# Lapis-Hong/wide_deep

Measured on NVIDIA H100. Metric: CTR examples/sec (train step), higher is better.
Workload: dtype bf16x3 (fp32 operands split into bf16 hi+lo, 3 tensor-core products, fp32 accumulate; 2^-16)

## Files before the change

### wide_deep_b200/csrc/gemm_bf16.cu

```cuda
#include <cuda.h>
#include <stdlib.h>

#include <algorithm>
#include <type_traits>

#include "common.cuh"
#include "gemm.cuh"
#include "wgmma_ptx.cuh"

namespace wd {

namespace {

constexpr int QBM = 128;
constexpr int QBN = 128;
constexpr int QNST = 3;
constexpr int QBK = 64;
constexpr int Q_THREADS = 384;

struct QMaps {
    CUtensorMap a_hi[kMaxSegs], a_lo[kMaxSegs];
    CUtensorMap b_hi, b_lo;
};
struct QSegs { int n; int k[kMaxSegs]; int koff[kMaxSegs]; };

__device__ unsigned long long g_probe[32 * 8];
__device__ __forceinline__ unsigned long long gtime() { unsigned long long t; asm volatile("mov.u64 %0, %globaltimer;" : "=l"(t)); return t; }
#define PROBE(i) do { if (probe >= 0 && blockIdx.x == 0 && (threadIdx.x & 127) == 0) g_probe[probe * 8 + (i)] = gtime(); } while (0)

template <int MODE>
__global__ void __launch_bounds__(Q_THREADS, 1) tc_gemm_bf16_kernel(const __grid_constant__ QMaps maps, const QSegs segs, int M, int N, int ktot,
                                                                   int ksplit_len, int nsplit, Epi ep, int probe) {
    extern __shared__ uint8_t smem_raw[];
    uint8_t* base = reinterpret_cast<uint8_t*>((reinterpret_cast<uintptr_t>(smem_raw) + 1023) & ~uintptr_t(1023));
    constexpr bool A_MN = MODE == EPI_WGRAD;
    constexpr bool B_MN = MODE == EPI_FWD || MODE == EPI_WGRAD;
    constexpr int A_BYTES = QBM * 128, B_BYTES = QBN * 128;
    constexpr int STAGE_BYTES = 2 * (A_BYTES + B_BYTES);
    auto a_hi = [&](int s) { return base + s * STAGE_BYTES; };
    auto a_lo = [&](int s) { return base + s * STAGE_BYTES + A_BYTES; };
    auto b_hi = [&](int s) { return base + s * STAGE_BYTES + 2 * A_BYTES; };
    auto b_lo = [&](int s) { return base + s * STAGE_BYTES + 2 * A_BYTES + B_BYTES; };
    uint64_t* bars = reinterpret_cast<uint64_t*>(base + QNST * STAGE_BYTES);
    uint64_t* full = bars; uint64_t* empty = bars + QNST;
    float* epi_vec = reinterpret_cast<float*>(base + QNST * STAGE_BYTES + 64);

    const int warp = threadIdx.x >> 5, lane = threadIdx.x & 31, wg = threadIdx.x >> 7;
    const int tiles_n = (N + QBN - 1) / QBN, tiles_m = (M + QBM - 1) / QBM;
    const int ntiles = tiles_n * tiles_m * nsplit;
    int nkb_all = 0;
    for (int s = 0; s < segs.n; ++s) nkb_all += (segs.k[s] + QBK - 1) / QBK;
    auto tile_range = [&](int tile, int& m0, int& n0, int& z, int& kbeg, int& nkb) {
        z = tile / (tiles_n * tiles_m);
        int r = tile % (tiles_n * tiles_m);
        m0 = (r / tiles_n) * QBM;
        n0 = (r % tiles_n) * QBN;
        kbeg = 0;
        nkb = nkb_all;
        if (MODE == EPI_WGRAD) {
            kbeg = z * ksplit_len;
            int kend = min(ktot, kbeg + ksplit_len);
            nkb = kend > kbeg ? (kend - kbeg + QBK - 1) / QBK : 0;
        }
    };

    if (threadIdx.x == 0) {
        for (int s = 0; s < QNST; ++s) { mbar_init(&full[s], 1); mbar_init(&empty[s], 8); }
        asm volatile("fence.mbarrier_init.release.cluster;" ::: "memory");
    }
    __syncthreads();

    if (wg == 0) {
        reg_dealloc<40>();
        PROBE(0);
        if (warp == 0 && lane == 0) {
            int g = 0;
            for (int tile = blockIdx.x; tile < ntiles; tile += gridDim.x) {
                int m0, n0, z, kbeg, nkb;
                tile_range(tile, m0, n0, z, kbeg, nkb);
                int seg = 0, kin = 0;
                for (int kb = 0; kb < nkb; ++kb, ++g) {
                    const int s = g % QNST, it = g / QNST;
                    if (it > 0) mbar_wait(&empty[s], (it - 1) & 1);
                    int ka, kbcoord;
                    if (MODE == EPI_WGRAD) { ka = kbeg + kb * QBK; kbcoord = ka; }
                    else {
                        if (kin >= segs.k[seg]) { ++seg; kin = 0; }
                        ka = kin; kbcoord = segs.koff[seg] + kin;
                        kin += QBK;
                    }
                    mbar_expect_tx(&full[s], 2 * (A_BYTES + B_BYTES));
                    if (!A_MN) {
                        tma_load_2d(a_hi(s), &maps.a_hi[seg], &full[s], ka, m0);
                        tma_load_2d(a_lo(s), &maps.a_lo[seg], &full[s], ka, m0);
                    } else {
#pragma unroll
                        for (int i = 0; i < QBM / 64; ++i) {
                            tma_load_2d(a_hi(s) + i * 8192, &maps.a_hi[seg], &full[s], m0 + 64 * i, ka);
                            tma_load_2d(a_lo(s) + i * 8192, &maps.a_lo[seg], &full[s], m0 + 64 * i, ka);
                        }
                    }
                    if (!B_MN) {
                        tma_load_2d(b_hi(s), &maps.b_hi, &full[s], kbcoord, n0);
                        tma_load_2d(b_lo(s), &maps.b_lo, &full[s], kbcoord, n0);
                    } else {
#pragma unroll
                        for (int i = 0; i < QBN / 64; ++i) {
                            tma_load_2d(b_hi(s) + i * 8192, &maps.b_hi, &full[s], n0 + 64 * i, kbcoord);
                            tma_load_2d(b_lo(s) + i * 8192, &maps.b_lo, &full[s], n0 + 64 * i, kbcoord);
                        }
                    }
                }
            }
        }
    } else {
        reg_alloc<232>();
        const int cw = wg - 1, cwarp = warp - 4;
        constexpr uint32_t a_step = A_MN ? 2048u : 32u, b_step = B_MN ? 2048u : 32u;
        constexpr int TA = A_MN ? 1 : 0, TB = B_MN ? 1 : 0;
        float d[QBN / 2];
        int g = 0, use = 0;
        for (int tile = blockIdx.x; tile < ntiles; tile += gridDim.x) {
            int m0, n0, z, kbeg, nkb;
            tile_range(tile, m0, n0, z, kbeg, nkb);
            if (nkb == 0) {
#pragma unroll
                for (int i = 0; i < QBN / 2; ++i) d[i] = 0.f;
            }
            const int ct = threadIdx.x - 128;
            float pre[2] = {0.f, 0.f};
            if (MODE == EPI_FWD) {
#pragma unroll
                for (int i = 0; i < 2; ++i) {
                    const int v = ct + 256 * i, c = n0 + (v & 127);
                    const bool in = c < ep.n_logical;
                    if (v < 128) pre[i] = in ? __ldg(ep.bias + c) : 0.f;
                    else if (v < 256) pre[i] = (in && ep.bn) ? __ldg(ep.gamma + c) * 0.99950037468777f : 1.f;
                    else if (v < 384) pre[i] = (in && ep.bn) ? __ldg(ep.beta + c) : 0.f;
                }
            }
            int prev = -1;
            for (int kb = 0; kb < nkb; ++kb, ++g) {
                const int s = g % QNST, it = g / QNST;
                mbar_wait(&full[s], it & 1);
                if (g == 0) PROBE(1);
                const uint32_t sa_hi = smem_u32(a_hi(s)) + cw * 8192, sa_lo = smem_u32(a_lo(s)) + cw * 8192;
                const uint32_t sb_hi = smem_u32(b_hi(s)), sb_lo = smem_u32(b_lo(s));
                wgmma_fence();
#pragma unroll
                for (int k = 0; k < QBK / 16; ++k) {
                    const uint64_t da_hi = A_MN ? make_desc_mn(sa_hi + k * a_step) : make_desc(sa_hi + k * a_step);
                    const uint64_t da_lo = A_MN ? make_desc_mn(sa_lo + k * a_step) : make_desc(sa_lo + k * a_step);
                    const uint64_t db_hi = B_MN ? make_desc_mn(sb_hi + k * b_step) : make_desc(sb_hi + k * b_step);
                    const uint64_t db_lo = B_MN ? make_desc_mn(sb_lo + k * b_step) : make_desc(sb_lo + k * b_step);
                    wgmma_bf16<TA, TB>(d, da_lo, db_hi, (kb > 0 || k > 0) ? 1u : 0u);
                    wgmma_bf16<TA, TB>(d, da_hi, db_lo, 1u);
                    wgmma_bf16<TA, TB>(d, da_hi, db_hi, 1u);
                }
                wgmma_commit();
                if (prev >= 0) {
                    wgmma_wait<1>();
                    if (lane == 0) mbar_arrive(&empty[prev]);
                }
                prev = s;
            }
            wgmma_wait<0>();
            if (prev >= 0 && lane == 0) mbar_arrive(&empty[prev]);
            if (cwarp == 0) PROBE(use == 0 ? 2 : 3);
            const float* ev = epi_vec + (use & 1) * 384;
            if (MODE == EPI_FWD) {
                epi_vec[(use & 1) * 384 + ct] = pre[0];
                if (ct < 128) epi_vec[(use & 1) * 384 + ct + 256] = pre[1];
                bar_sync(1, 256);
            }

            const int r0 = m0 + cw * 64 + (warp & 3) * 16 + (lane >> 2);
            const int cq = 2 * (lane & 3);
            auto epilogue = [&](auto relu) {
                constexpr bool RELU = decltype(relu)::value;
                uint32_t qh[2][2] = {}, ql[2][2] = {};
#pragma unroll
                for (int j = 0; j < QBN / 8; ++j) {
                    const int c = n0 + 8 * j + cq;
                    if (n0 + 8 * j < N) {
                        if (MODE == EPI_FWD) {
                            const bool in0 = c < ep.n_logical, in1 = c + 1 < ep.n_logical;
                            const int cl = 8 * j + cq;
                            const float b0 = ev[cl], b1 = ev[cl + 1], g0 = ev[128 + cl], g1 = ev[129 + cl], e0 = ev[256 + cl], e1 = ev[257 + cl];
#pragma unroll
                            for (int hh = 0; hh < 2; ++hh) {
                                const int r = r0 + 8 * hh;
                                if (r >= M) continue;
                                const bool rv = r < ep.m_valid;
                                float a0 = 0.f, a1 = 0.f, h0 = 0.f, h1 = 0.f;
                                if (rv && in0) { a0 = RELU ? fmaxf(d[4 * j + 2 * hh] + b0, 0.f) : act_fwd(ep.act, d[4 * j + 2 * hh] + b0); h0 = fmaf(a0, g0, e0); }
                                if (rv && in1) { a1 = RELU ? fmaxf(d[4 * j + 2 * hh + 1] + b1, 0.f) : act_fwd(ep.act, d[4 * j + 2 * hh + 1] + b1); h1 = fmaf(a1, g1, e1); }
                                const int64_t o = (int64_t)r * ep.ldh + c;
                                if (ep.A_out != ep.H_out) *reinterpret_cast<float2*>(ep.A_out + o) = make_float2(a0, a1);
                                if (ep.H_out) *reinterpret_cast<float2*>(ep.H_out + o) = make_float2(h0, h1);
                                split_pair(h0, h1, qh[j & 1][hh], ql[j & 1][hh]);
                            }
                            if (j & 1) {
                                const int q = lane & 3, src = (lane & ~3) + 2 * (q & 1);
                                const int64_t cp = n0 + 16 * (j >> 1) + 4 * q;
#pragma unroll
                                for (int hh = 0; hh < 2; ++hh) {
                                    uint2 vh, vl;
                                    const uint32_t h0a = __shfl_sync(0xffffffffu, qh[0][hh], src), h1a = __shfl_sync(0xffffffffu, qh[1][hh], src);
                                    const uint32_t h0b = __shfl_sync(0xffffffffu, qh[0][hh], src + 1), h1b = __shfl_sync(0xffffffffu, qh[1][hh], src + 1);
                                    const uint32_t l0a = __shfl_sync(0xffffffffu, ql[0][hh], src), l1a = __shfl_sync(0xffffffffu, ql[1][hh], src);
                                    const uint32_t l0b = __shfl_sync(0xffffffffu, ql[0][hh], src + 1), l1b = __shfl_sync(0xffffffffu, ql[1][hh], src + 1);
                                    vh.x = q < 2 ? h0a : h1a; vh.y = q < 2 ? h0b : h1b;
                                    vl.x = q < 2 ? l0a : l1a; vl.y = q < 2 ? l0b : l1b;
                                    const int r = r0 + 8 * hh;
                                    if (r >= M) continue;
                                    const int64_t o = (int64_t)r * ep.ldh + cp;
                                    *reinterpret_cast<uint2*>(ep.Hs_hi + o) = vh;
                                    *reinterpret_cast<uint2*>(ep.Hs_lo + o) = vl;
                                }
                            }
                        } else {
                            float* Cb = ep.C + (MODE == EPI_WGRAD ? (int64_t)z * ep.split_stride : 0);
#pragma unroll
                            for (int hh = 0; hh < 2; ++hh) {
                                const int r = r0 + 8 * hh;
                                if (r >= M) continue;
                                float2* pc = reinterpret_cast<float2*>(Cb + (int64_t)r * ep.ldc + c);
                                float2 o = make_float2(d[4 * j + 2 * hh], d[4 * j + 2 * hh + 1]);
                                if (MODE == EPI_STORE && ep.accumulate) { const float2 p = *pc; o.x += p.x; o.y += p.y; }
                                *pc = o;
                            }
                        }
                    }
                }
            };
            if (MODE == EPI_FWD && ep.act == WD_ACT_RELU) epilogue(std::true_type{});
            else epilogue(std::false_type{});
            if (cwarp == 0) PROBE(use == 0 ? 4 : 5);
            ++use;
        }
    }
}

int g_probe_slot = 0;

template <int MODE>
int launch_q(WdModel* m, const QMaps& maps, const QSegs& segs, int M, int N, int ktot, int splits, int ksplit_len, const Epi& ep) {
    constexpr int smem = QNST * 2 * (QBM * 128 + QBN * 128) + 1024 + 64 + 2 * 384 * 4;
    static bool configured = false;
    static int num_sms = 0;
    if (!configured) {
        WD_CUDA(cudaFuncSetAttribute(tc_gemm_bf16_kernel<MODE>, cudaFuncAttributeMaxDynamicSharedMemorySize, smem));
        WD_CUDA(cudaDeviceGetAttribute(&num_sms, cudaDevAttrMultiProcessorCount, m->device));
        configured = true;
    }
    const int nsplit = MODE == EPI_WGRAD ? splits : 1;
    const int ntiles = ((N + QBN - 1) / QBN) * ((M + QBM - 1) / QBM) * nsplit;
    static const bool probe_on = getenv("WD_GEMM_PROBE") != nullptr;
    const int probe = probe_on ? (g_probe_slot++ & 31) : -1;
    tc_gemm_bf16_kernel<MODE><<<ntiles < num_sms ? ntiles : num_sms, Q_THREADS, smem, m->stream>>>(maps, segs, M, N, ktot, ksplit_len, nsplit, ep, probe);
    m->launches++;
    WD_CUDA(cudaGetLastError());
    return WD_OK;
}

}

extern "C" int wd_debug_gemm_probe(unsigned long long* out) {
    cudaDeviceSynchronize();
    cudaError_t e = cudaMemcpyFromSymbol(out, g_probe, sizeof(unsigned long long) * 32 * 8);
    g_probe_slot = 0;
    return e == cudaSuccess ? 0 : -1;
}

int tc_gemm_bf16(WdModel* m, int mode, const GemmA& A, const GemmB& B, int M, int N, const Epi& ep, int splits, int ksplit_len) {
    constexpr CUtensorMapDataType BF16 = CU_TENSOR_MAP_DATA_TYPE_BFLOAT16;
    if (N % 32 != 0 || A.n > kMaxSegs || !B.hi || !B.lo) { set_error("bf16 GEMM engine: unsupported operands"); return WD_EUNSUPPORTED; }
    QMaps maps;
    QSegs segs{};
    segs.n = A.n;
    int rc, ktot = 0;
    const bool a_mn = mode == EPI_WGRAD, b_mn = mode == EPI_FWD || mode == EPI_WGRAD;
    for (int s = 0; s < A.n; ++s) {
        if (!A.hi[s] || !A.lo[s]) { set_error("bf16 GEMM engine: operand without hi/lo copies"); return WD_EINVAL; }
        if (!a_mn) {
            if ((rc = make_tensor_map(&maps.a_hi[s], BF16, A.hi[s], M, A.k[s], A.ld[s], QBM))) return rc;
            if ((rc = make_tensor_map(&maps.a_lo[s], BF16, A.lo[s], M, A.k[s], A.ld[s], QBM))) return rc;
        } else {
            if ((rc = make_tensor_map(&maps.a_hi[s], BF16, A.hi[s], A.k[s], M, A.ld[s], 64))) return rc;
            if ((rc = make_tensor_map(&maps.a_lo[s], BF16, A.lo[s], A.k[s], M, A.ld[s], 64))) return rc;
        }
        segs.k[s] = A.k[s]; segs.koff[s] = ktot;
        ktot += A.k[s];
    }
    for (int s = A.n; s < kMaxSegs; ++s) { maps.a_hi[s] = maps.a_hi[0]; maps.a_lo[s] = maps.a_lo[0]; }
    if (!b_mn) {
        if ((rc = make_tensor_map(&maps.b_hi, BF16, B.hi, N, ktot, B.ld, QBN))) return rc;
        if ((rc = make_tensor_map(&maps.b_lo, BF16, B.lo, N, ktot, B.ld, QBN))) return rc;
    } else {
        if ((rc = make_tensor_map(&maps.b_hi, BF16, B.hi, ktot, N, B.ld, 64))) return rc;
        if ((rc = make_tensor_map(&maps.b_lo, BF16, B.lo, ktot, N, B.ld, 64))) return rc;
    }
    if (mode == EPI_WGRAD) ksplit_len = (ksplit_len + QBK - 1) / QBK * QBK;
    if (mode == EPI_FWD && (!ep.Hs_hi || !ep.Hs_lo)) { set_error("bf16 GEMM engine: epilogue without hi/lo outputs"); return WD_EINVAL; }
    if (mode == EPI_FWD) return launch_q<EPI_FWD>(m, maps, segs, M, N, ktot, splits, ksplit_len, ep);
    if (mode == EPI_STORE) return launch_q<EPI_STORE>(m, maps, segs, M, N, ktot, splits, ksplit_len, ep);
    return launch_q<EPI_WGRAD>(m, maps, segs, M, N, ktot, splits, ksplit_len, ep);
}

}
```

### wide_deep_b200/csrc/wgmma_ptx.cuh

```cuda
#pragma once
#include <cuda.h>
#include <stdint.h>

namespace wd {

__device__ __forceinline__ uint32_t smem_u32(const void* p) { return (uint32_t)__cvta_generic_to_shared(p); }
__device__ __forceinline__ void mbar_init(uint64_t* bar, uint32_t count) {
    asm volatile("mbarrier.init.shared::cta.b64 [%0], %1;" ::"r"(smem_u32(bar)), "r"(count));
}
__device__ __forceinline__ void mbar_expect_tx(uint64_t* bar, uint32_t bytes) {
    asm volatile("mbarrier.arrive.expect_tx.shared::cta.b64 _, [%0], %1;" ::"r"(smem_u32(bar)), "r"(bytes) : "memory");
}
__device__ __forceinline__ void mbar_arrive(uint64_t* bar) {
    asm volatile("mbarrier.arrive.shared::cta.b64 _, [%0];" ::"r"(smem_u32(bar)) : "memory");
}
__device__ __forceinline__ void mbar_wait(uint64_t* bar, uint32_t parity) {
    asm volatile(
        "{\n\t.reg .pred p;\n\t"
        "WAIT_LOOP:\n\t"
        "mbarrier.try_wait.parity.shared::cta.b64 p, [%0], %1;\n\t"
        "@p bra WAIT_DONE;\n\t"
        "bra WAIT_LOOP;\n\t"
        "WAIT_DONE:\n\t}" ::"r"(smem_u32(bar)), "r"(parity) : "memory");
}
__device__ __forceinline__ void tma_load_2d(void* dst, const CUtensorMap* map, uint64_t* bar, int c0, int c1) {
    asm volatile("cp.async.bulk.tensor.2d.shared::cluster.global.mbarrier::complete_tx::bytes [%0], [%1, {%3, %4}], [%2];"
                 ::"r"(smem_u32(dst)), "l"(reinterpret_cast<uint64_t>(map)), "r"(smem_u32(bar)), "r"(c0), "r"(c1) : "memory");
}

__device__ __forceinline__ void bar_sync(int id, int n) { asm volatile("bar.sync %0, %1;" ::"r"(id), "r"(n) : "memory"); }

template <int N> __device__ __forceinline__ void reg_dealloc() { asm volatile("setmaxnreg.dec.sync.aligned.u32 %0;" ::"n"(N)); }
template <int N> __device__ __forceinline__ void reg_alloc() { asm volatile("setmaxnreg.inc.sync.aligned.u32 %0;" ::"n"(N)); }

__device__ __forceinline__ void wgmma_fence() { asm volatile("wgmma.fence.sync.aligned;" ::: "memory"); }
__device__ __forceinline__ void wgmma_commit() { asm volatile("wgmma.commit_group.sync.aligned;" ::: "memory"); }
template <int N> __device__ __forceinline__ void wgmma_wait() { asm volatile("wgmma.wait_group.sync.aligned %0;" ::"n"(N) : "memory"); }

__device__ __forceinline__ uint64_t make_desc(uint32_t saddr) {
    uint64_t d = 0;
    d |= (uint64_t)((saddr >> 4) & 0x3FFF);
    d |= (uint64_t)1 << 16;
    d |= (uint64_t)(1024 >> 4) << 32;
    d |= (uint64_t)1 << 62;
    return d;
}

__device__ __forceinline__ uint64_t make_desc_mn(uint32_t saddr) {
    uint64_t d = 0;
    d |= (uint64_t)((saddr >> 4) & 0x3FFF);
    d |= (uint64_t)(8192 >> 4) << 16;
    d |= (uint64_t)(1024 >> 4) << 32;
    d |= (uint64_t)1 << 62;
    return d;
}

template <int TA, int TB>
__device__ __forceinline__ void wgmma_bf16(float (&d)[64], uint64_t desc_a, uint64_t desc_b, uint32_t accumulate) {
    asm volatile(
        "{\n\t.reg .pred p;\n\tsetp.ne.b32 p, %66, 0;\n\t"
        "wgmma.mma_async.sync.aligned.m64n128k16.f32.bf16.bf16 {"
        "%0, %1, %2, %3, %4, %5, %6, %7, %8, %9, %10, %11, %12, %13, %14, %15, %16, %17, %18, %19, %20, %21, %22, %23, %24, %25, "
        "%26, %27, %28, %29, %30, %31, %32, %33, %34, %35, %36, %37, %38, %39, %40, %41, %42, %43, %44, %45, %46, %47, %48, %49, "
        "%50, %51, %52, %53, %54, %55, %56, %57, %58, %59, %60, %61, %62, %63}, "
        "%64, %65, p, 1, 1, %67, %68;\n\t}"
        : "+f"(d[0]), "+f"(d[1]), "+f"(d[2]), "+f"(d[3]), "+f"(d[4]), "+f"(d[5]), "+f"(d[6]), "+f"(d[7]),
          "+f"(d[8]), "+f"(d[9]), "+f"(d[10]), "+f"(d[11]), "+f"(d[12]), "+f"(d[13]), "+f"(d[14]), "+f"(d[15]),
          "+f"(d[16]), "+f"(d[17]), "+f"(d[18]), "+f"(d[19]), "+f"(d[20]), "+f"(d[21]), "+f"(d[22]), "+f"(d[23]),
          "+f"(d[24]), "+f"(d[25]), "+f"(d[26]), "+f"(d[27]), "+f"(d[28]), "+f"(d[29]), "+f"(d[30]), "+f"(d[31]),
          "+f"(d[32]), "+f"(d[33]), "+f"(d[34]), "+f"(d[35]), "+f"(d[36]), "+f"(d[37]), "+f"(d[38]), "+f"(d[39]),
          "+f"(d[40]), "+f"(d[41]), "+f"(d[42]), "+f"(d[43]), "+f"(d[44]), "+f"(d[45]), "+f"(d[46]), "+f"(d[47]),
          "+f"(d[48]), "+f"(d[49]), "+f"(d[50]), "+f"(d[51]), "+f"(d[52]), "+f"(d[53]), "+f"(d[54]), "+f"(d[55]),
          "+f"(d[56]), "+f"(d[57]), "+f"(d[58]), "+f"(d[59]), "+f"(d[60]), "+f"(d[61]), "+f"(d[62]), "+f"(d[63])
        : "l"(desc_a), "l"(desc_b), "r"(accumulate), "n"(TA), "n"(TB));
}
__device__ __forceinline__ void wgmma_tf32(float (&d)[64], uint64_t desc_a, uint64_t desc_b, uint32_t accumulate) {
    asm volatile(
        "{\n\t.reg .pred p;\n\tsetp.ne.b32 p, %66, 0;\n\t"
        "wgmma.mma_async.sync.aligned.m64n128k8.f32.tf32.tf32 {"
        "%0, %1, %2, %3, %4, %5, %6, %7, %8, %9, %10, %11, %12, %13, %14, %15, %16, %17, %18, %19, %20, %21, %22, %23, %24, %25, "
        "%26, %27, %28, %29, %30, %31, %32, %33, %34, %35, %36, %37, %38, %39, %40, %41, %42, %43, %44, %45, %46, %47, %48, %49, "
        "%50, %51, %52, %53, %54, %55, %56, %57, %58, %59, %60, %61, %62, %63}, "
        "%64, %65, p, 1, 1;\n\t}"
        : "+f"(d[0]), "+f"(d[1]), "+f"(d[2]), "+f"(d[3]), "+f"(d[4]), "+f"(d[5]), "+f"(d[6]), "+f"(d[7]),
          "+f"(d[8]), "+f"(d[9]), "+f"(d[10]), "+f"(d[11]), "+f"(d[12]), "+f"(d[13]), "+f"(d[14]), "+f"(d[15]),
          "+f"(d[16]), "+f"(d[17]), "+f"(d[18]), "+f"(d[19]), "+f"(d[20]), "+f"(d[21]), "+f"(d[22]), "+f"(d[23]),
          "+f"(d[24]), "+f"(d[25]), "+f"(d[26]), "+f"(d[27]), "+f"(d[28]), "+f"(d[29]), "+f"(d[30]), "+f"(d[31]),
          "+f"(d[32]), "+f"(d[33]), "+f"(d[34]), "+f"(d[35]), "+f"(d[36]), "+f"(d[37]), "+f"(d[38]), "+f"(d[39]),
          "+f"(d[40]), "+f"(d[41]), "+f"(d[42]), "+f"(d[43]), "+f"(d[44]), "+f"(d[45]), "+f"(d[46]), "+f"(d[47]),
          "+f"(d[48]), "+f"(d[49]), "+f"(d[50]), "+f"(d[51]), "+f"(d[52]), "+f"(d[53]), "+f"(d[54]), "+f"(d[55]),
          "+f"(d[56]), "+f"(d[57]), "+f"(d[58]), "+f"(d[59]), "+f"(d[60]), "+f"(d[61]), "+f"(d[62]), "+f"(d[63])
        : "l"(desc_a), "l"(desc_b), "r"(accumulate));
}

}
```

Before: 10.42 million.

## Stage forward GEMM epilogue outputs in shared memory and write via TMA stores

The forward-mode epilogue now writes activations, BN outputs and the bf16 hi/lo splits into swizzled shared-memory tiles, reusing freed pipeline stages. It then issues TMA tensor stores instead of per-thread scattered global stores and warp shuffles. Release of the held stage's empty barrier is deferred until the next tile's first k-block, so the bulk stores overlap with the next mainloop. This adds barrier syncs, extra tensor maps and delicate stage-reuse logic, which risk stalling the producer or creating races.

Result: faster. 10.53 million, median of 6 (+1.1%).

```diff
diff --git a/wide_deep_b200/csrc/gemm_bf16.cu b/wide_deep_b200/csrc/gemm_bf16.cu
--- a/wide_deep_b200/csrc/gemm_bf16.cu
+++ b/wide_deep_b200/csrc/gemm_bf16.cu
@@ -22,6 +22,10 @@
     CUtensorMap a_hi[kMaxSegs], a_lo[kMaxSegs];
     CUtensorMap b_hi, b_lo;
 };
+struct QFwdMaps : QMaps {
+    CUtensorMap hs_hi, hs_lo, a_out, h_out;
+};
+template <int MODE> using QMapsOf = std::conditional_t<MODE == EPI_FWD, QFwdMaps, QMaps>;
 struct QSegs { int n; int k[kMaxSegs]; int koff[kMaxSegs]; };
 
 __device__ unsigned long long g_probe[32 * 8];
@@ -29,7 +33,7 @@
 #define PROBE(i) do { if (probe >= 0 && blockIdx.x == 0 && (threadIdx.x & 127) == 0) g_probe[probe * 8 + (i)] = gtime(); } while (0)
 
 template <int MODE>
-__global__ void __launch_bounds__(Q_THREADS, 1) tc_gemm_bf16_kernel(const __grid_constant__ QMaps maps, const QSegs segs, int M, int N, int ktot,
+__global__ void __launch_bounds__(Q_THREADS, 1) tc_gemm_bf16_kernel(const __grid_constant__ QMapsOf<MODE> maps, const QSegs segs, int M, int N, int ktot,
                                                                    int ksplit_len, int nsplit, Epi ep, int probe) {
     extern __shared__ uint8_t smem_raw[];
     uint8_t* base = reinterpret_cast<uint8_t*>((reinterpret_cast<uintptr_t>(smem_raw) + 1023) & ~uintptr_t(1023));
@@ -120,6 +124,7 @@
         constexpr int TA = A_MN ? 1 : 0, TB = B_MN ? 1 : 0;
         float d[QBN / 2];
         int g = 0, use = 0;
+        int held = -1;
         for (int tile = blockIdx.x; tile < ntiles; tile += gridDim.x) {
             int m0, n0, z, kbeg, nkb;
             tile_range(tile, m0, n0, z, kbeg, nkb);
@@ -158,6 +163,14 @@
                     wgmma_bf16<TA, TB>(d, da_hi, db_hi, 1u);
                 }
                 wgmma_commit();
+                if (MODE == EPI_FWD && kb == 0 && held >= 0) {
+                    if (ct == 0) {
+                        bulk_wait_read<0>();
+                        mbar_arrive(&empty[held]);
+                        if (use == 1) PROBE(6);
+                    }
+                    held = -1;
+                }
                 if (prev >= 0) {
                     wgmma_wait<1>();
                     if (lane == 0) mbar_arrive(&empty[prev]);
@@ -165,87 +178,119 @@
                 prev = s;
             }
             wgmma_wait<0>();
-            if (prev >= 0 && lane == 0) mbar_arrive(&empty[prev]);
+            if (MODE != EPI_FWD && prev >= 0 && lane == 0) mbar_arrive(&empty[prev]);
             if (cwarp == 0) PROBE(use == 0 ? 2 : 3);
-            const float* ev = epi_vec + (use & 1) * 384;
-            if (MODE == EPI_FWD) {
+            const int cq = 2 * (lane & 3);
+            if constexpr (MODE == EPI_FWD) {
+                const float* ev = epi_vec + (use & 1) * 384;
                 epi_vec[(use & 1) * 384 + ct] = pre[0];
                 if (ct < 128) epi_vec[(use & 1) * 384 + ct + 256] = pre[1];
                 bar_sync(1, 256);
-            }
-
-            const int r0 = m0 + cw * 64 + (warp & 3) * 16 + (lane >> 2);
-            const int cq = 2 * (lane & 3);
-            auto epilogue = [&](auto relu) {
-                constexpr bool RELU = decltype(relu)::value;
-                uint32_t qh[2][2] = {}, ql[2][2] = {};
+
+                const int rl = cw * 64 + (warp & 3) * 16 + (lane >> 2);
+                const bool rv[2] = {m0 + rl < ep.m_valid, m0 + rl + 8 < ep.m_valid};
+                auto valid = [&](int j, int hh, int e) { return rv[hh] && n0 + 8 * j + cq + e < ep.n_logical; };
+                auto activate = [&](auto relu) {
+                    constexpr bool RELU = decltype(relu)::value;
+#pragma unroll
+                    for (int j = 0; j < QBN / 8; ++j)
+#pragma unroll
+                        for (int hh = 0; hh < 2; ++hh)
+#pragma unroll
+                            for (int e = 0; e < 2; ++e) {
+                                float& x = d[4 * j + 2 * hh + e];
+                                const float2 b = *reinterpret_cast<const float2*>(ev + 8 * j + cq);
+                                const float be = e ? b.y : b.x;
+                                x = valid(j, hh, e) ? (RELU ? fmaxf(x + be, 0.f) : act_fwd(ep.act, x + be)) : 0.f;
+                            }
+                };
+                if (ep.act == WD_ACT_RELU) activate(std::true_type{});
+                else activate(std::false_type{});
+                auto h_of = [&](int j, int hh) {
+                    const float2 g = *reinterpret_cast<const float2*>(ev + 128 + 8 * j + cq), e = *reinterpret_cast<const float2*>(ev + 256 + 8 * j + cq);
+                    return make_float2(valid(j, hh, 0) ? fmaf(d[4 * j + 2 * hh], g.x, e.x) : 0.f,
+                                       valid(j, hh, 1) ? fmaf(d[4 * j + 2 * hh + 1], g.y, e.y) : 0.f);
+                };
+                const bool last_tile = tile + (int)gridDim.x >= ntiles;
+                auto stage_of = [&](int r) { return base + (last_tile ? (prev + r) % QNST : prev) * STAGE_BYTES; };
+                auto at = [&](int r, int box, int row, int byte) {
+                    return smem_u32(stage_of(r)) + box * 16384 + row * 128 + (((byte >> 4) ^ (row & 7)) << 4) + (byte & 15);
+                };
+                auto hand_over = [&](int r, const CUtensorMap* map01, const CUtensorMap* map23, bool bf16, bool last) {
+                    fence_proxy_async_smem();
+                    bar_sync(1, 256);
+                    if (ct == 0) {
+#pragma unroll
+                        for (int i = 0; i < 4; ++i) {
+                            const int c = n0 + (bf16 ? 64 * (i & 1) : 32 * i);
+                            if (c < N) tma_store_2d(i < 2 ? map01 : map23, stage_of(r) + i * 16384, c, m0);
+                        }
+                        bulk_commit();
+                        if (last) PROBE(use == 0 ? 4 : 5);
+                        else if (!last_tile) bulk_wait_read<0>();
+                    }
+                    if (!last && !last_tile) bar_sync(1, 256);
+                };
+                auto stage_f32 = [&](int r, bool h) {
+#pragma unroll
+                    for (int j = 0; j < QBN / 8; ++j)
+#pragma unroll
+                        for (int hh = 0; hh < 2; ++hh) {
+                            st_shared(at(r, j >> 2, rl + 8 * hh, 4 * (8 * (j & 3) + cq)), h ? h_of(j, hh) : make_float2(d[4 * j + 2 * hh], d[4 * j + 2 * hh + 1]));
+                        }
+                };
+                const bool st_a = ep.A_out != ep.H_out, st_h = ep.H_out != nullptr;
+#pragma unroll
+                for (int j = 0; j < QBN / 8; ++j)
+#pragma unroll
+                    for (int hh = 0; hh < 2; ++hh) {
+                        uint32_t hi, lo;
+                        const float2 h = h_of(j, hh);
+                        split_pair(h.x, h.y, hi, lo);
+                        const int byte = 2 * (8 * (j & 7) + cq);
+                        st_shared(at(0, j >> 3, rl + 8 * hh, byte), hi);
+                        st_shared(at(0, 2 + (j >> 3), rl + 8 * hh, byte), lo);
+                    }
+                hand_over(0, &maps.hs_hi, &maps.hs_lo, true, !st_a && !st_h);
+                if (st_a) { stage_f32(1, false); hand_over(1, &maps.a_out, &maps.a_out, false, !st_h); }
+                if (st_h) { stage_f32(2, true); hand_over(2, &maps.h_out, &maps.h_out, false, true); }
+                if (!last_tile) {
+                    if (cwarp != 0 && lane == 0) mbar_arrive(&empty[prev]);
+                    held = prev;
+                }
+            } else {
+                const int r0 = m0 + cw * 64 + (warp & 3) * 16 + (lane >> 2);
 #pragma unroll
                 for (int j = 0; j < QBN / 8; ++j) {
                     const int c = n0 + 8 * j + cq;
                     if (n0 + 8 * j < N) {
-                        if (MODE == EPI_FWD) {
-                            const bool in0 = c < ep.n_logical, in1 = c + 1 < ep.n_logical;
-                            const int cl = 8 * j + cq;
-                            const float b0 = ev[cl], b1 = ev[cl + 1], g0 = ev[128 + cl], g1 = ev[129 + cl], e0 = ev[256 + cl], e1 = ev[257 + cl];
-#pragma unroll
-                            for (int hh = 0; hh < 2; ++hh) {
-                                const int r = r0 + 8 * hh;
-                                if (r >= M) continue;
-                                const bool rv = r < ep.m_valid;
-                                float a0 = 0.f, a1 = 0.f, h0 = 0.f, h1 = 0.f;
-                                if (rv && in0) { a0 = RELU ? fmaxf(d[4 * j + 2 * hh] + b0, 0.f) : act_fwd(ep.act, d[4 * j + 2 * hh] + b0); h0 = fmaf(a0, g0, e0); }
-                                if (rv && in1) { a1 = RELU ? fmaxf(d[4 * j + 2 * hh + 1] + b1, 0.f) : act_fwd(ep.act, d[4 * j + 2 * hh + 1] + b1); h1 = fmaf(a1, g1, e1); }
-                                const int64_t o = (int64_t)r * ep.ldh + c;
-                                if (ep.A_out != ep.H_out) *reinterpret_cast<float2*>(ep.A_out + o) = make_float2(a0, a1);
-                                if (ep.H_out) *reinterpret_cast<float2*>(ep.H_out + o) = make_float2(h0, h1);
-                                split_pair(h0, h1, qh[j & 1][hh], ql[j & 1][hh]);
-                            }
-                            if (j & 1) {
-                                const int q = lane & 3, src = (lane & ~3) + 2 * (q & 1);
-                                const int64_t cp = n0 + 16 * (j >> 1) + 4 * q;
-#pragma unroll
-                                for (int hh = 0; hh < 2; ++hh) {
-                                    uint2 vh, vl;
-                                    const uint32_t h0a = __shfl_sync(0xffffffffu, qh[0][hh], src), h1a = __shfl_sync(0xffffffffu, qh[1][hh], src);
-                                    const uint32_t h0b = __shfl_sync(0xffffffffu, qh[0][hh], src + 1), h1b = __shfl_sync(0xffffffffu, qh[1][hh], src + 1);
-                                    const uint32_t l0a = __shfl_sync(0xffffffffu, ql[0][hh], src), l1a = __shfl_sync(0xffffffffu, ql[1][hh], src);
-                                    const uint32_t l0b = __shfl_sync(0xffffffffu, ql[0][hh], src + 1), l1b = __shfl_sync(0xffffffffu, ql[1][hh], src + 1);
-                                    vh.x = q < 2 ? h0a : h1a; vh.y = q < 2 ? h0b : h1b;
-                                    vl.x = q < 2 ? l0a : l1a; vl.y = q < 2 ? l0b : l1b;
-                                    const int r = r0 + 8 * hh;
-                                    if (r >= M) continue;
-                                    const int64_t o = (int64_t)r * ep.ldh + cp;
-                                    *reinterpret_cast<uint2*>(ep.Hs_hi + o) = vh;
-                                    *reinterpret_cast<uint2*>(ep.Hs_lo + o) = vl;
-                                }
-                            }
-                        } else {
-                            float* Cb = ep.C + (MODE == EPI_WGRAD ? (int64_t)z * ep.split_stride : 0);
-#pragma unroll
-                            for (int hh = 0; hh < 2; ++hh) {
-                                const int r = r0 + 8 * hh;
-                                if (r >= M) continue;
-                                float2* pc = reinterpret_cast<float2*>(Cb + (int64_t)r * ep.ldc + c);
-                                float2 o = make_float2(d[4 * j + 2 * hh], d[4 * j + 2 * hh + 1]);
-                                if (MODE == EPI_STORE && ep.accumulate) { const float2 p = *pc; o.x += p.x; o.y += p.y; }
-                                *pc = o;
-                            }
-                        }
-                    }
-                }
-            };
-            if (MODE == EPI_FWD && ep.act == WD_ACT_RELU) epilogue(std::true_type{});
-            else epilogue(std::false_type{});
-            if (cwarp == 0) PROBE(use == 0 ? 4 : 5);
+                        float* Cb = ep.C + (MODE == EPI_WGRAD ? (int64_t)z * ep.split_stride : 0);
+#pragma unroll
+                        for (int hh = 0; hh < 2; ++hh) {
+                            const int r = r0 + 8 * hh;
+                            if (r >= M) continue;
+                            float2* pc = reinterpret_cast<float2*>(Cb + (int64_t)r * ep.ldc + c);
+                            float2 o = make_float2(d[4 * j + 2 * hh], d[4 * j + 2 * hh + 1]);
+                            if (MODE == EPI_STORE && ep.accumulate) { const float2 p = *pc; o.x += p.x; o.y += p.y; }
+                            *pc = o;
+                        }
+                    }
+                }
+                if (cwarp == 0) PROBE(use == 0 ? 4 : 5);
+            }
             ++use;
         }
+        if (MODE == EPI_FWD && threadIdx.x == 128) {
+            bulk_wait<0>();
+            if (use == 1) PROBE(6);
+        }
     }
 }
 
 int g_probe_slot = 0;
 
 template <int MODE>
-int launch_q(WdModel* m, const QMaps& maps, const QSegs& segs, int M, int N, int ktot, int splits, int ksplit_len, const Epi& ep) {
+int launch_q(WdModel* m, const QMapsOf<MODE>& maps, const QSegs& segs, int M, int N, int ktot, int splits, int ksplit_len, const Epi& ep) {
     constexpr int smem = QNST * 2 * (QBM * 128 + QBN * 128) + 1024 + 64 + 2 * 384 * 4;
     static bool configured = false;
     static int num_sms = 0;
@@ -276,7 +321,7 @@
 int tc_gemm_bf16(WdModel* m, int mode, const GemmA& A, const GemmB& B, int M, int N, const Epi& ep, int splits, int ksplit_len) {
     constexpr CUtensorMapDataType BF16 = CU_TENSOR_MAP_DATA_TYPE_BFLOAT16;
     if (N % 32 != 0 || A.n > kMaxSegs || !B.hi || !B.lo) { set_error("bf16 GEMM engine: unsupported operands"); return WD_EUNSUPPORTED; }
-    QMaps maps;
+    QFwdMaps maps;
     QSegs segs{};
     segs.n = A.n;
     int rc, ktot = 0;
@@ -302,8 +347,16 @@
         if ((rc = make_tensor_map(&maps.b_lo, BF16, B.lo, ktot, N, B.ld, 64))) return rc;
     }
     if (mode == EPI_WGRAD) ksplit_len = (ksplit_len + QBK - 1) / QBK * QBK;
-    if (mode == EPI_FWD && (!ep.Hs_hi || !ep.Hs_lo)) { set_error("bf16 GEMM engine: epilogue without hi/lo outputs"); return WD_EINVAL; }
-    if (mode == EPI_FWD) return launch_q<EPI_FWD>(m, maps, segs, M, N, ktot, splits, ksplit_len, ep);
+    if (mode == EPI_FWD) {
+        if (!ep.Hs_hi || !ep.Hs_lo || !ep.A_out) { set_error("bf16 GEMM engine: epilogue without hi/lo outputs"); return WD_EINVAL; }
+        constexpr CUtensorMapDataType F32 = CU_TENSOR_MAP_DATA_TYPE_FLOAT32;
+        if ((rc = make_tensor_map(&maps.hs_hi, BF16, ep.Hs_hi, M, N, ep.ldh, QBM))) return rc;
+        if ((rc = make_tensor_map(&maps.hs_lo, BF16, ep.Hs_lo, M, N, ep.ldh, QBM))) return rc;
+        maps.a_out = maps.h_out = maps.hs_hi;
+        if (ep.A_out != ep.H_out && (rc = make_tensor_map(&maps.a_out, F32, ep.A_out, M, N, ep.ldh, QBM))) return rc;
+        if (ep.H_out && (rc = make_tensor_map(&maps.h_out, F32, ep.H_out, M, N, ep.ldh, QBM))) return rc;
+        return launch_q<EPI_FWD>(m, maps, segs, M, N, ktot, splits, ksplit_len, ep);
+    }
     if (mode == EPI_STORE) return launch_q<EPI_STORE>(m, maps, segs, M, N, ktot, splits, ksplit_len, ep);
     return launch_q<EPI_WGRAD>(m, maps, segs, M, N, ktot, splits, ksplit_len, ep);
 }
diff --git a/wide_deep_b200/csrc/wgmma_ptx.cuh b/wide_deep_b200/csrc/wgmma_ptx.cuh
--- a/wide_deep_b200/csrc/wgmma_ptx.cuh
+++ b/wide_deep_b200/csrc/wgmma_ptx.cuh
@@ -27,6 +27,16 @@
     asm volatile("cp.async.bulk.tensor.2d.shared::cluster.global.mbarrier::complete_tx::bytes [%0], [%1, {%3, %4}], [%2];"
                  ::"r"(smem_u32(dst)), "l"(reinterpret_cast<uint64_t>(map)), "r"(smem_u32(bar)), "r"(c0), "r"(c1) : "memory");
 }
+__device__ __forceinline__ void tma_store_2d(const CUtensorMap* map, const void* src, int c0, int c1) {
+    asm volatile("cp.async.bulk.tensor.2d.global.shared::cta.bulk_group [%0, {%2, %3}], [%1];"
+                 ::"l"(reinterpret_cast<uint64_t>(map)), "r"(smem_u32(src)), "r"(c0), "r"(c1) : "memory");
+}
+__device__ __forceinline__ void bulk_commit() { asm volatile("cp.async.bulk.commit_group;" ::: "memory"); }
+template <int N> __device__ __forceinline__ void bulk_wait_read() { asm volatile("cp.async.bulk.wait_group.read %0;" ::"n"(N) : "memory"); }
+template <int N> __device__ __forceinline__ void bulk_wait() { asm volatile("cp.async.bulk.wait_group %0;" ::"n"(N) : "memory"); }
+__device__ __forceinline__ void st_shared(uint32_t addr, uint32_t v) { asm volatile("st.shared.b32 [%0], %1;" ::"r"(addr), "r"(v) : "memory"); }
+__device__ __forceinline__ void st_shared(uint32_t addr, float2 v) { asm volatile("st.shared.v2.f32 [%0], {%1, %2};" ::"r"(addr), "f"(v.x), "f"(v.y) : "memory"); }
+__device__ __forceinline__ void fence_proxy_async_smem() { asm volatile("fence.proxy.async.shared::cta;" ::: "memory"); }
 
 __device__ __forceinline__ void bar_sync(int id, int n) { asm volatile("bar.sync %0, %1;" ::"r"(id), "r"(n) : "memory"); }
 
```
